# Mingqj/OcRFDet

Measured on AMD Instinct MI355X. Metric: BEV voxels/sec + rendered views/sec, 6-cam 256x704, higher is better.
Workload: dtype f32

## Files before the change

ocrfdet_amd/csrc/common.hip:

```cpp
#include <hip/hip_runtime.h>

#include <mutex>
#include <vector>

#include "launch.h"
#include "ocrf_hip.h"

namespace {

struct Timer {
  int kernel_id = 0;
  std::vector<hipEvent_t> start, stop;
  int used = 0;
};

std::mutex g_mu;
std::vector<Timer*> g_armed;
volatile int g_n_armed = 0;

}

namespace {

__global__ void zero_words_kernel(unsigned* __restrict__ dst, size_t n_words) {
  const size_t i = (size_t)blockIdx.x * blockDim.x + threadIdx.x;
  if (i < n_words) dst[i] = 0u;
}

__global__ void diag_stamp_kernel(unsigned long long* __restrict__ slot) { *slot = wall_clock64(); }

__global__ void diag_where_kernel(unsigned* __restrict__ out, int spin) {
  unsigned xcc, hw;
  asm volatile("s_getreg_b32 %0, hwreg(HW_REG_XCC_ID)" : "=s"(xcc));
  asm volatile("s_getreg_b32 %0, hwreg(HW_REG_HW_ID)" : "=s"(hw));
  const unsigned long long t0 = wall_clock64();
  while (wall_clock64() - t0 < (unsigned long long)spin) __builtin_amdgcn_s_sleep(8);
  if (threadIdx.x == 0) out[blockIdx.x] = ((xcc & 0xFu) << 16) | (hw & 0xFFFFu);
}

}

namespace ocrf {

hipError_t zero_async(void* dst, size_t bytes, hipStream_t stream) {
  const size_t n = bytes / 4;
  if (n == 0) return hipSuccess;
  hipLaunchKernelGGL(zero_words_kernel, dim3((unsigned)((n + 255) / 256)), dim3(256), 0, stream,
                     static_cast<unsigned*>(dst), n);
  return hipGetLastError();
}

bool timer_next(int kernel_id, hipEvent_t* start, hipEvent_t* stop) {
  if (!g_n_armed) return false;
  std::lock_guard<std::mutex> lk(g_mu);
  for (Timer* t : g_armed) {
    if (t->kernel_id != kernel_id || t->used >= (int)t->start.size()) continue;
    *start = t->start[t->used];
    *stop = t->stop[t->used];
    ++t->used;
    return true;
  }
  return false;
}

}

extern "C" {

const char* ocrf_version(void) { return "ocrf_hip 0.1 gfx950"; }

int ocrf_diag_stamp(unsigned long long* slot, void* stream) {
  hipLaunchKernelGGL(diag_stamp_kernel, dim3(1), dim3(1), 0, static_cast<hipStream_t>(stream), slot);
  return (int)hipGetLastError();
}

int ocrf_diag_where(int n_blocks, unsigned* out, int spin_ticks, void* stream) {
  if (n_blocks <= 0 || !out) return (int)hipErrorInvalidValue;
  hipLaunchKernelGGL(diag_where_kernel, dim3(n_blocks), dim3(64), 0, static_cast<hipStream_t>(stream), out, spin_ticks);
  return (int)hipGetLastError();
}

const char* ocrf_kernel_name(int kernel_id) {
  switch (kernel_id) {
    case OCRF_K_BEV_POOL_FWD: return "bev_pool_tile_kernel<false>";
    case OCRF_K_BEV_POOL_INTERVAL: return "bev_pool_interval_kernel";
    case OCRF_K_BEV_POOL_MFMA: return "bev_pool_mfma_kernel<*>";
    case OCRF_K_BEV_POOL_PANEL: return "bev_pool_panel_kernel<*>";
    case OCRF_K_BEV_POOL_CELL_WEIGHTS: return "bev_pool_cell_weights_kernel";
    case OCRF_K_BEV_POOL_GRAD: return "bev_pool_grad_vec_kernel";
    case OCRF_K_RASTER_PREPROCESS: return "raster_preprocess_kernel";
    case OCRF_K_RASTER_BLEND: return "raster_blend_kernel<false, false, *>";
    case OCRF_K_RASTER_BLEND_BWD: return "raster_blend_kernel<false, true, true>";
    case OCRF_K_RASTER_PRE_BWD: return "raster_preprocess_backward_kernel<false>";
    case OCRF_K_RASTER_GATHER: return "raster_scatter_kernel";
    case OCRF_K_RASTER_PLAN_UPDATE: return "raster_plan_update_kernel";
    case OCRF_K_RASTER_BLEND_SORTED: return "raster_blend_sorted_kernel<*>";
    case OCRF_K_RASTER_SCAN: return "raster_bucket_scan_kernel";
    case OCRF_K_HOA_STATS: return "hoa_channel_stats_kernel";
    case OCRF_K_HOA_MASK_GATE: return "hoa_mask_gate_kernel";
    case OCRF_K_HOA_HEIGHT_MAX: return "hoa_height_max_kernel";
    case OCRF_K_HOA_HEIGHT_GATE: return "hoa_height_gate_kernel";
    case OCRF_K_HOA_UNET_BLOCK: return "hoa_unet_block_kernel";
    case OCRF_K_HOA_OUT_CONV: return "hoa_gated_conv1x1_kernel";
    case OCRF_K_HOA1_ATTN: return "hoa1_attention_upsample_kernel";
    case OCRF_K_HOA1_UP: return "(unused)";
    case OCRF_K_HOA1_Q: return "(unused)";
    case OCRF_K_HOA1_KV: return "hoa1_kv_kernel";
    case OCRF_K_HOA_DW3X3: return "hoa_dw3x3_kernel";
    case OCRF_K_HOA_DW3X3_WGRAD: return "hoa_dw3x3_wgrad_kernel";
    case OCRF_K_LSS_KEYS: return "lss_keys_hist_kernel";
    case OCRF_K_RADIX_HIST: return "radix_hist_kernel";
    case OCRF_K_SCAN: return "scan_apply_kernel<*>";
    case OCRF_K_RADIX_SCATTER: return "radix_scatter_kernel<*>";
    case OCRF_K_LSS_BOUNDS: return "lss_intervals_kernel";
    case OCRF_K_LSS_EMIT: return "(unused)";
    case OCRF_K_HT_COUNT: return "ht_valid_kernel";
    case OCRF_K_HT_EMIT: return "ht_emit_kernel";
    case OCRF_K_HT_PROJECT: return "ht_project_kernel";
    case OCRF_K_NECK_PREFILTER: return "neck_prefilter_kernel";
    case OCRF_K_NECK_SAMPLE: return "neck_pillar_sample_mean_kernel<*>";
    case OCRF_K_NECK_RETAIN: return "neck_retain_scatter_kernel";
    case OCRF_K_NECK_HEADS: return "neck_gauss_heads_kernel";
    case OCRF_K_NECK_NERF_ALPHA: return "neck_nerf_alpha_kernel";
    case OCRF_K_NECK_NERF_RENDER: return "neck_nerf_render_kernel";
    case OCRF_K_NECK_FUSION: return "neck_dual_fusion_kernel<*>";
    case OCRF_K_NECK_PLANE_PASS: return "neck_plane_pass_kernel<*>";
    case OCRF_K_NECK_CHANNEL_MLP: return "neck_channel_mlp_kernel";
    case OCRF_K_NECK_SCALED_STATS: return "neck_scaled_channel_stats_kernel";
    case OCRF_K_NECK_CBAM_TAIL: return "neck_cbam_tail_kernel";
    case OCRF_K_LOSS_DEPTH_LABELS: return "depth_labels_kernel";
    case OCRF_K_LOSS_DS: return "ds_loss_partial_kernel";
    case OCRF_K_LOSS_FINAL: return "ds_loss_final_kernel / render_final_kernel";
    case OCRF_K_LOSS_DS_BWD: return "ds_loss_backward_kernel";
    case OCRF_K_LOSS_RENDER: return "render_tile_kernel";
    case OCRF_K_LOSS_RENDER_DEPTH: return "render_depth_kernel";
    case OCRF_K_LOSS_RENDER_BWD: return "render_backward_kernel";
    case OCRF_K_STEREO_COST_VOLUME: return "stereo_cost_volume_kernel";
    case OCRF_K_CH_ASSIGN: return "ch_assign_kernel";
    case OCRF_K_CH_HEATMAP: return "ch_heatmap_kernel";
    case OCRF_K_CH_HM_LOSS: return "ch_hm_loss_partial_kernel";
    case OCRF_K_CH_FINAL: return "ch_hm_loss_final_kernel / ch_reg_loss_final_kernel";
    case OCRF_K_CH_HM_LOSS_BWD: return "ch_hm_loss_backward_kernel";
    case OCRF_K_CH_REG_LOSS: return "ch_reg_loss_partial_kernel";
    case OCRF_K_CH_REG_LOSS_BWD: return "ch_reg_loss_backward_kernel";
    case OCRF_K_CD_SELECT: return "cd_select_kernel";
    case OCRF_K_CD_MASK: return "cd_mask_kernel";
    case OCRF_K_CD_SCAN: return "cd_scan_kernel";
    case OCRF_K_CD_WRITE: return "cd_write_kernel";
    case OCRF_K_UPSAMPLE_CAT: return "upsample_cat_kernel<float, *>";
    case OCRF_K_UPSAMPLE_CAT_BWD: return "upsample_cat_backward_kernel<float>";
    case OCRF_K_ADD_RELU: return "binary_kernel<*, AddRelu>";
    case OCRF_K_ADD_RELU_BWD: return "binary_kernel<*, Threshold>";
    case OCRF_K_UPSAMPLE_ADD: return "upsample_add_kernel<*>";
    case OCRF_K_UPSAMPLE_ADD_BWD: return "upsample_add_backward_kernel";
    case OCRF_K_BEV_ALIGN: return "bev_align_kernel<float, *>";
    case OCRF_K_BEV_ALIGN_BWD: return "bev_align_backward_kernel<float>";
    case OCRF_K_OPTIM_SQNORM: return "optim_grad_sqnorm_kernel";
    case OCRF_K_OPTIM_NORM_FINAL: return "optim_norm_final_kernel";
    case OCRF_K_OPTIM_STEP: return "optim_step_kernel";
    case OCRF_K_ADD_RELU_BF16: return "binary_bf16_kernel<*, AddRelu>";
    case OCRF_K_ADD_RELU_BWD_BF16: return "binary_bf16_kernel<*, Threshold>";
    case OCRF_K_UPSAMPLE_ADD_BF16: return "upsample_add_bf16_kernel<*>";
    case OCRF_K_UPSAMPLE_ADD_BWD_BF16: return "upsample_add_backward_bf16_kernel";
    case OCRF_K_UPSAMPLE_CAT_BF16: return "upsample_cat_kernel<unsigned short, *>";
    case OCRF_K_UPSAMPLE_CAT_BWD_BF16: return "upsample_cat_backward_kernel<unsigned short>";
    case OCRF_K_BEV_ALIGN_BF16: return "bev_align_kernel<unsigned short, *>";
    case OCRF_K_BEV_ALIGN_BWD_BF16: return "bev_align_backward_kernel<unsigned short>";
    case OCRF_K_STEREO_PACK_BF16: return "stereo_pack_bf16_kernel";
    case OCRF_K_STEREO_COST_VOLUME_BF16: return "stereo_cost_volume_bf16_kernel";
    case OCRF_K_BN_STATS: return "bn_stats_kernel<float, *>";
    case OCRF_K_BN_FINALIZE: return "bn_finalize_kernel";
    case OCRF_K_BN_ACT_FWD: return "bn_act_forward_kernel<float, *>";
    case OCRF_K_BN_ACT_BWD_REDUCE: return "bn_act_backward_reduce_kernel<float, *>";
    case OCRF_K_BN_ACT_BWD: return "bn_act_backward_kernel<float, *>";
    case OCRF_K_BN_STATS_BF16: return "bn_stats_kernel<unsigned short, *>";
    case OCRF_K_BN_ACT_FWD_BF16: return "bn_act_forward_kernel<unsigned short, *>";
    case OCRF_K_BN_ACT_BWD_REDUCE_BF16: return "bn_act_backward_reduce_kernel<unsigned short, *>";
    case OCRF_K_BN_ACT_BWD_BF16: return "bn_act_backward_kernel<unsigned short, *>";
    case OCRF_K_FRAME_POSES: return "frame_poses_kernel";
    case OCRF_K_IMAGE_PREP_HORIZONTAL: return "image_prep_horizontal_kernel";
    case OCRF_K_IMAGE_PREP_VERTICAL: return "image_prep_vertical_kernel";
    case OCRF_K_IMAGE_PREP_EPILOGUE: return "image_prep_epilogue_kernel";
    case OCRF_K_POINT_LABELS_MARK: return "point_labels_mark_kernel";
    case OCRF_K_POINT_LABELS_RESOLVE: return "point_labels_resolve_kernel";
    case OCRF_K_DEFORM_IM2COL: return "deform_im2col_kernel";
    case OCRF_K_DEFORM_COL2IM: return "deform_col2im_kernel";
    case OCRF_K_GROUP_CORR: return "group_corr_forward_kernel<*>";
    case OCRF_K_GROUP_CORR_GRAD_LEFT: return "group_corr_grad_left_kernel<*>";
    case OCRF_K_GROUP_CORR_GRAD_RIGHT: return "group_corr_grad_right_kernel<*>";
    case OCRF_K_KD_PARTIAL: return "kd_partial_kernel";
    case OCRF_K_KD_FINAL: return "kd_final_kernel";
    case OCRF_K_KD_BWD: return "kd_backward_kernel";
    case OCRF_K_RASTER_BLEND_BWD_DEPTH: return "raster_blend_kernel<false, true, true, true, true>";
    case OCRF_K_RASTER_PRE_BWD_DEPTH: return "raster_preprocess_backward_kernel<true>";
    case OCRF_K_HOA1_ATTN_TRAIN: return "hoa1_attention_train_kernel";
    case OCRF_K_HOA1_UP_GRAD: return "hoa1_up_grad_kernel";
    case OCRF_K_HOA1_ATTN_GRAD: return "hoa1_attn_grad_kernel";
    case OCRF_K_HOA1_KV_GRAD: return "hoa1_kv_grad_kernel";
    case OCRF_K_HOA1_TOKEN_GRAD: return "hoa1_token_grad_kernel";
    case OCRF_K_HOA1_PIXEL_GRAD: return "hoa1_pixel_grad_kernel";
    case OCRF_K_HOA1_WEIGHT_SUM: return "hoa1_weight_sum_kernel";
    default: return "";
  }
}

int ocrf_timer_create(int capacity, void** timer_out) {
  if (capacity <= 0 || !timer_out) return (int)hipErrorInvalidValue;
  Timer* t = new Timer();
  t->start.resize(capacity);
  t->stop.resize(capacity);
  for (int i = 0; i < capacity; ++i) {
    hipError_t e = hipEventCreate(&t->start[i]);
    if (e == hipSuccess) e = hipEventCreate(&t->stop[i]);
    if (e != hipSuccess) { delete t; return (int)e; }
  }
  *timer_out = t;
  return 0;
}

int ocrf_timer_arm(void* timer, int kernel_id) {
  std::lock_guard<std::mutex> lk(g_mu);
  Timer* t = static_cast<Timer*>(timer);
  if (!t) {
    g_armed.clear();
  } else {
    t->kernel_id = kernel_id;
    t->used = 0;
    bool present = false;
    for (Timer* q : g_armed) present = present || (q == t);
    if (!present) g_armed.push_back(t);
  }
  g_n_armed = (int)g_armed.size();
  return 0;
}

int ocrf_timer_read(void* timer, float* ms_out, int capacity, int* count_out) {
  Timer* t = static_cast<Timer*>(timer);
  if (!t || !count_out) return (int)hipErrorInvalidValue;
  int n = 0;
  {
    std::lock_guard<std::mutex> lk(g_mu);
    n = t->used;
  }
  if (n > capacity) n = capacity;
  for (int i = 0; i < n; ++i) {
    hipError_t e = hipEventSynchronize(t->stop[i]);
    if (e == hipSuccess) e = hipEventElapsedTime(&ms_out[i], t->start[i], t->stop[i]);
    if (e != hipSuccess) return (int)e;
  }
  *count_out = n;
  return 0;
}

int ocrf_stream_create(const uint32_t* cu_mask, int n_words, int priority, void** stream_out) {
  if (!stream_out || n_words < 0) return (int)hipErrorInvalidValue;
  hipStream_t s = nullptr;
  hipError_t e;
  if (cu_mask && n_words > 0) {
    e = hipExtStreamCreateWithCUMask(&s, (uint32_t)n_words, cu_mask);
  } else {
    e = hipStreamCreateWithPriority(&s, hipStreamNonBlocking, priority);
  }
  if (e != hipSuccess) return (int)e;
  *stream_out = s;
  return 0;
}

int ocrf_stream_write_value32(int* ptr, int value, ocrf_stream_t stream) {
  if (!ptr) return (int)hipErrorInvalidValue;
  return (int)hipStreamWriteValue32(static_cast<hipStream_t>(stream), ptr, (uint32_t)value, 0);
}

int ocrf_graph_node_census(void* graph, int* n_kernel, int* n_memset, int* n_memcpy, int* n_other) {
  if (!graph || !n_kernel || !n_memset || !n_memcpy || !n_other) return (int)hipErrorInvalidValue;
  size_t n = 0;
  hipError_t e = hipGraphGetNodes(static_cast<hipGraph_t>(graph), nullptr, &n);
  if (e != hipSuccess) return (int)e;
  std::vector<hipGraphNode_t> nodes(n);
  if (n) {
    e = hipGraphGetNodes(static_cast<hipGraph_t>(graph), nodes.data(), &n);
    if (e != hipSuccess) return (int)e;
  }
  *n_kernel = *n_memset = *n_memcpy = *n_other = 0;
  for (size_t i = 0; i < n; ++i) {
    hipGraphNodeType t;
    e = hipGraphNodeGetType(nodes[i], &t);
    if (e != hipSuccess) return (int)e;
    if (t == hipGraphNodeTypeKernel) ++*n_kernel;
    else if (t == hipGraphNodeTypeMemset) ++*n_memset;
    else if (t == hipGraphNodeTypeMemcpy) ++*n_memcpy;
    else ++*n_other;
  }
  return 0;
}

int ocrf_stream_destroy(void* stream) {
  return stream ? (int)hipStreamDestroy(static_cast<hipStream_t>(stream)) : 0;
}

int ocrf_timer_destroy(void* timer) {
  Timer* t = static_cast<Timer*>(timer);
  if (!t) return 0;
  {
    std::lock_guard<std::mutex> lk(g_mu);
    for (size_t i = 0; i < g_armed.size(); ++i)
      if (g_armed[i] == t) { g_armed.erase(g_armed.begin() + i); break; }
    g_n_armed = (int)g_armed.size();
  }
  for (auto e : t->start) (void)hipEventDestroy(e);
  for (auto e : t->stop) (void)hipEventDestroy(e);
  delete t;
  return 0;
}

}
```

ocrfdet_amd/csrc/hoa.hip:

```cpp
#include <hip/hip_runtime.h>

#include <algorithm>

#include "hoa1_common.h"
#include "launch.h"
#include "ocrf_hip.h"

namespace {

constexpr int kBlock = 256;
int g_mg_groups = 0, g_mg_threads = kBlock, g_stats_threads = kBlock;

__device__ __forceinline__ float sigmoidf_(float v) { return 1.0f / (1.0f + __expf(-v)); }

__global__ __launch_bounds__(kBlock) void hoa_channel_stats_kernel(const float* __restrict__ x, int C,
                                                                   long plane, float* __restrict__ stats) {
  OCRF_MAIN_CHAIN_PRIO();
  const long pix = (long)blockIdx.x * blockDim.x + threadIdx.x;
  const int b = blockIdx.y;
  if (pix >= plane) return;
  const float* p = x + (long)b * C * plane + pix;
  float sum = 0.f, mx = -INFINITY;
  int c = 0;
  for (; c + 16 <= C; c += 16) {
    float v[16];
#pragma unroll
    for (int u = 0; u < 16; ++u) v[u] = p[(long)(c + u) * plane];
#pragma unroll
    for (int u = 0; u < 16; ++u) {
      sum += v[u];
      mx = fmaxf(mx, v[u]);
    }
  }
  for (; c < C; ++c) {
    const float v = p[(long)c * plane];
    sum += v;
    mx = fmaxf(mx, v);
  }
  stats[((long)b * 2 + 0) * plane + pix] = sum / (float)C;
  stats[((long)b * 2 + 1) * plane + pix] = mx;
}

template <int VEC, int KT, bool FAST = false>
__global__ __launch_bounds__(kBlock) void hoa_mask_gate_kernel(
    const float* __restrict__ x, const float* __restrict__ stats, const float* __restrict__ opacity_bev,
    const float* __restrict__ conv_w, int k_rt, int C, int Y, int X, int groups, int n_rows,
    float* __restrict__ mask, float* __restrict__ gated) {
  OCRF_MAIN_CHAIN_PRIO();
  const int k = KT ? KT : k_rt;
  const int nt = (int)blockDim.x;
  extern __shared__ __attribute__((aligned(16))) float s_dyn[];
  const int r = k / 2, tw = FAST ? X + 8 : ((VEC == 4) ? ((X + k - 1 + 3) & ~3) : (X + k - 1));
  constexpr int PL = FAST ? 1 : 0;
  float* s_w = s_dyn;
  float* s_s = s_dyn + ((VEC == 4) ? ((2 * k * k + 3) & ~3) : 2 * k * k);
  const long plane = (long)Y * X;
  const int b = blockIdx.z / groups, g = blockIdx.z % groups;
  const long p0 = (long)blockIdx.x * nt * VEC;
  const int row0 = (int)(p0 / X) - r;
  for (int i = threadIdx.x; i < 2 * k * k; i += nt) s_w[i] = conv_w[i];
  const long pix_e = p0 + (long)threadIdx.x * VEC;
  const int cpg_e = (C + groups - 1) / groups;
  const int c0_e = g * cpg_e, c1_e = min(C, c0_e + cpg_e);
  float4 first[5];
  const bool pre = (VEC == 4) && gated && pix_e < plane && c0_e + 5 <= c1_e;
  if constexpr (VEC == 4) {
    if (pre) {
      const float* pe = x + (long)b * C * plane + pix_e;
#pragma unroll
      for (int u = 0; u < 5; ++u) first[u] = *reinterpret_cast<const float4*>(pe + (long)(c0_e + u) * plane);
    }
  }
  if constexpr (FAST) {
    const int n_items = 2 * n_rows * 64, x4 = X >> 2;
    float4* s_s4 = reinterpret_cast<float4*>(s_s);
    const int tw4 = tw >> 2;
    for (int i0 = 0; i0 < n_items; i0 += 8 * nt) {
      float4 v[8];
#pragma unroll
      for (int u = 0; u < 8; ++u) {
        const int i = min(i0 + u * nt + (int)threadIdx.x, n_items - 1);
        const int rp = i >> 6, c4 = min(i & 63, x4 - 1);
        const int ch = rp >= n_rows ? 1 : 0, y = row0 + rp - ch * n_rows;
        v[u] = *reinterpret_cast<const float4*>(stats + ((long)b * 2 + ch) * plane + (long)min(max(y, 0), Y - 1) * X + 4 * c4);
      }
#pragma unroll
      for (int u = 0; u < 8; ++u) {
        const int i = i0 + u * nt + (int)threadIdx.x;
        const int rp = i >> 6, c4 = i & 63;
        const int ch = rp >= n_rows ? 1 : 0, y = row0 + rp - ch * n_rows;
        const bool in = y >= 0 && y < Y;
        if (i < n_items && c4 < x4) s_s4[rp * tw4 + 1 + c4] = in ? v[u] : make_float4(0.f, 0.f, 0.f, 0.f);
      }
    }
    for (int i = threadIdx.x; i < 2 * n_rows * 2; i += nt)
      s_s4[(i >> 1) * tw4 + ((i & 1) ? 1 + x4 : 0)] = make_float4(0.f, 0.f, 0.f, 0.f);
  } else {
  const int n_stage = 2 * n_rows * tw;
  for (int i0 = 0; i0 < n_stage; i0 += 8 * nt) {
    float v[8];
#pragma unroll
    for (int u = 0; u < 8; ++u) {
      const int i = i0 + u * nt + threadIdx.x;
      const int ch = i / (n_rows * tw), rem = i % (n_rows * tw);
      const int y = row0 + rem / tw, xx = rem % tw - r;
      v[u] = (i < n_stage && y >= 0 && y < Y && xx >= 0 && xx < X)
                 ? stats[((long)b * 2 + ch) * plane + (long)y * X + xx] : 0.f;
    }
#pragma unroll
    for (int u = 0; u < 8; ++u) {
      const int i = i0 + u * nt + threadIdx.x;
      if (i < n_stage) s_s[i] = v[u];
    }
  }
  }
  __syncthreads();
  const long pix = p0 + (long)threadIdx.x * VEC;
  if (pix >= plane) return;
  const int yy = (int)(pix / X), xx = (int)(pix % X);
  const int ly = yy - row0 - r;
  float acc[VEC];
#pragma unroll
  for (int e = 0; e < VEC; ++e) acc[e] = 0.f;
  if constexpr (KT > 0) {
#pragma unroll
    for (int ch = 0; ch < 2; ++ch) {
#pragma unroll
      for (int i = 0; i < KT; ++i) {
        const float* row = s_s + (ch * n_rows + ly + i) * tw + xx;
        const float* wr = s_w + (ch * KT + i) * KT;
        float win[(KT + VEC - 1 + 3) & ~3];
        if constexpr (VEC == 4) {
          const float4* row4 = reinterpret_cast<const float4*>(row);
#pragma unroll
          for (int j = 0; j < (KT + VEC - 1 + 3) / 4; ++j) {
            const float4 q4 = row4[j];
            win[4 * j] = q4.x; win[4 * j + 1] = q4.y; win[4 * j + 2] = q4.z; win[4 * j + 3] = q4.w;
          }
        } else {
#pragma unroll
          for (int j = 0; j < KT + VEC - 1; ++j) win[j] = row[j];
        }
#pragma unroll
        for (int j = 0; j < KT; ++j) {
          const float w = wr[j];
#pragma unroll
          for (int e = 0; e < VEC; ++e) acc[e] = fmaf(win[j + e + PL], w, acc[e]);
        }
      }
    }
  } else {
    for (int ch = 0; ch < 2; ++ch)
      for (int i = 0; i < k; ++i) {
        const float* row = s_s + (ch * n_rows + ly + i) * tw + xx;
        const float* wr = s_w + (ch * k + i) * k;
        for (int j = 0; j < k; ++j) {
          const float w = wr[j];
#pragma unroll
          for (int e = 0; e < VEC; ++e) acc[e] = fmaf(row[j + e], w, acc[e]);
        }
      }
  }
  float m[VEC];
#pragma unroll
  for (int e = 0; e < VEC; ++e) m[e] = sigmoidf_(acc[e] + opacity_bev[(long)b * plane + pix + e]);
  if (g == 0) {
#pragma unroll
    for (int e = 0; e < VEC; ++e) mask[(long)b * plane + pix + e] = m[e];
  }
  if (gated) {
    const int cpg = (C + groups - 1) / groups;
    const int c0 = g * cpg, c1 = min(C, c0 + cpg);
    const float* p = x + (long)b * C * plane + pix;
    float* q = gated + (long)b * C * plane + pix;
    if constexpr (VEC == 4) {
      int c = c0;
      if (pre) {
#pragma unroll
        for (int u = 0; u < 5; ++u)
          *reinterpret_cast<float4*>(q + (long)(c + u) * plane) =
              make_float4(first[u].x * m[0], first[u].y * m[1], first[u].z * m[2], first[u].w * m[3]);
        c += 5;
      }
      for (; c + 5 <= c1; c += 5) {
        float4 v[5];
#pragma unroll
        for (int u = 0; u < 5; ++u) v[u] = *reinterpret_cast<const float4*>(p + (long)(c + u) * plane);
#pragma unroll
        for (int u = 0; u < 5; ++u)
          *reinterpret_cast<float4*>(q + (long)(c + u) * plane) =
              make_float4(v[u].x * m[0], v[u].y * m[1], v[u].z * m[2], v[u].w * m[3]);
      }
      for (; c < c1; ++c) {
        const float4 v = *reinterpret_cast<const float4*>(p + (long)c * plane);
        *reinterpret_cast<float4*>(q + (long)c * plane) = make_float4(v.x * m[0], v.y * m[1], v.z * m[2], v.w * m[3]);
      }
    } else {
      int c = c0;
      for (; c + 10 <= c1; c += 10) {
        float v[10];
#pragma unroll
        for (int u = 0; u < 10; ++u) v[u] = p[(long)(c + u) * plane];
#pragma unroll
        for (int u = 0; u < 10; ++u) q[(long)(c + u) * plane] = v[u] * m[0];
      }
      for (; c < c1; ++c) q[(long)c * plane] = p[(long)c * plane] * m[0];
    }
  }
}

__global__ __launch_bounds__(kBlock) void hoa_height_max_kernel(const float* __restrict__ x, long plane,
                                                                int n_split, float* __restrict__ partial) {
  __shared__ float s_m[kBlock / 64];
  const long bc = blockIdx.y;
  const float* p = x + bc * plane;
  const long chunk = (plane + n_split - 1) / n_split;
  const long lo = (long)blockIdx.x * chunk, hi = min(lo + chunk, plane);
  float m = -INFINITY;
  for (long i = lo + threadIdx.x; i < hi; i += kBlock) m = fmaxf(m, p[i]);
  for (int off = 32; off > 0; off >>= 1) m = fmaxf(m, __shfl_down(m, off));
  if ((threadIdx.x & 63) == 0) s_m[threadIdx.x >> 6] = m;
  __syncthreads();
  if (threadIdx.x == 0) {
    for (int w = 1; w < kBlock / 64; ++w) m = fmaxf(m, s_m[w]);
    partial[bc * n_split + blockIdx.x] = m;
  }
}

__global__ __launch_bounds__(kBlock) void hoa_height_gate_kernel(
    const float* __restrict__ x, int C, int hid, long plane, int n_split, const float* __restrict__ partial,
    const float* __restrict__ w1, const float* __restrict__ w2, float* __restrict__ gate,
    float* __restrict__ gated) {
  __shared__ float s_max[64];
  __shared__ float s_hid[64];
  __shared__ float s_gate[64];
  const int b = blockIdx.y, tid = threadIdx.x;
  const int q = C / 4;
  if (tid < C) {
    float m = -INFINITY;
    for (int s = 0; s < n_split; ++s) m = fmaxf(m, partial[((long)b * C + tid) * n_split + s]);
    s_max[tid] = m;
  }
  __syncthreads();
  if (tid < 4 * hid) {
    const int g = tid / hid, h = tid % hid;
    float a = 0.f;
    for (int i = 0; i < q; ++i) a = fmaf(w1[(g * hid + h) * q + i], s_max[g * q + i], a);
    s_hid[tid] = fmaxf(a, 0.f);
  }
  __syncthreads();
  if (tid < C) {
    const int g = tid / q, o = tid % q;
    float a = 0.f;
    for (int h = 0; h < hid; ++h) a = fmaf(w2[(g * q + o) * hid + h], s_hid[g * hid + h], a);
    const float gt = sigmoidf_(a);
    s_gate[tid] = gt;
    if (blockIdx.x == 0) gate[(long)b * C + tid] = gt;
  }
  __syncthreads();
  if (!gated) return;
  const long pix = (long)blockIdx.x * kBlock + tid;
  if (pix >= plane) return;
  const float* p = x + (long)b * C * plane + pix;
  float* o = gated + (long)b * C * plane + pix;
  for (int c = 0; c < C; ++c) o[(long)c * plane] = p[(long)c * plane] * s_gate[c];
}

constexpr int kDwBand = 16;
__global__ __launch_bounds__(kBlock) void hoa_dw3x3_kernel(const float* __restrict__ x, const float* __restrict__ w,
                                                           const float* __restrict__ bias, int C, int Y, int X,
                                                           float* __restrict__ y) {
  const int bc = blockIdx.z, c = bc % C;
  const int xx = blockIdx.x * 64 + (threadIdx.x & 63), yy = blockIdx.y * 4 + (threadIdx.x >> 6);
  if (xx >= X || yy >= Y) return;
  const float* p = x + (long)bc * Y * X;
  float acc = bias ? bias[c] : 0.f;
#pragma unroll
  for (int i = 0; i < 3; ++i) {
    const int sy = yy + i - 1;
    if (sy < 0 || sy >= Y) continue;
#pragma unroll
    for (int j = 0; j < 3; ++j) {
      const int sx = xx + j - 1;
      if (sx < 0 || sx >= X) continue;
      acc = fmaf(w[c * 9 + i * 3 + j], p[(long)sy * X + sx], acc);
    }
  }
  y[(long)bc * Y * X + (long)yy * X + xx] = acc;
}

__global__ __launch_bounds__(kBlock) void hoa_dw3x3_wgrad_kernel(const float* __restrict__ x,
                                                                 const float* __restrict__ dy, int Y, int X,
                                                                 float* __restrict__ partial) {
  __shared__ float s_acc[kBlock / 64][10];
  const int bc = blockIdx.y, band = blockIdx.x;
  const float* px = x + (long)bc * Y * X;
  const float* pg = dy + (long)bc * Y * X;
  const int y0 = band * kDwBand, y1 = min(y0 + kDwBand, Y);
  float acc[10];
#pragma unroll
  for (int t = 0; t < 10; ++t) acc[t] = 0.f;
  for (int idx = threadIdx.x; idx < (y1 - y0) * X; idx += kBlock) {
    const int yy = y0 + idx / X, xx = idx % X;
    const float g = pg[(long)yy * X + xx];
    acc[9] += g;
#pragma unroll
    for (int i = 0; i < 3; ++i) {
      const int sy = yy + i - 1;
      if (sy < 0 || sy >= Y) continue;
#pragma unroll
      for (int j = 0; j < 3; ++j) {
        const int sx = xx + j - 1;
        if (sx < 0 || sx >= X) continue;
        acc[i * 3 + j] = fmaf(g, px[(long)sy * X + sx], acc[i * 3 + j]);
      }
    }
  }
#pragma unroll
  for (int t = 0; t < 10; ++t) {
    float v = acc[t];
    for (int off = 32; off > 0; off >>= 1) v += __shfl_down(v, off);
    if ((threadIdx.x & 63) == 0) s_acc[threadIdx.x >> 6][t] = v;
  }
  __syncthreads();
  if (threadIdx.x < 10) {
    float v = 0.f;
    for (int wv = 0; wv < kBlock / 64; ++wv) v += s_acc[wv][threadIdx.x];
    partial[((long)bc * gridDim.x + band) * 10 + threadIdx.x] = v;
  }
}

}

namespace ocrf {
void hoa_tune(int key, int value) {
  if (key == 20 && value >= 0) g_mg_groups = value;
  if (key == 21 && (value == 64 || value == 128 || value == 256)) g_mg_threads = value;
  if (key == 22 && (value == 64 || value == 128 || value == 256)) g_stats_threads = value;
}
}

extern "C" {

int ocrf_hoa_dw3x3(const float* x, const float* w, const float* bias, int B, int C, int Y, int X, float* y,
                   ocrf_stream_t stream_) {
  if (!x || !w || !y || B <= 0 || C <= 0 || Y <= 0 || X <= 0 || (long)B * C > 65535) return (int)hipErrorInvalidValue;
  ocrf::launch(OCRF_K_HOA_DW3X3, hoa_dw3x3_kernel, dim3((X + 63) / 64, (Y + 3) / 4, B * C), dim3(kBlock), 0,
               static_cast<hipStream_t>(stream_), x, w, bias, C, Y, X, y);
  return (int)hipGetLastError();
}

int ocrf_hoa_dw3x3_wgrad_bands(int Y) { return (Y + kDwBand - 1) / kDwBand; }

int ocrf_hoa_dw3x3_wgrad(const float* x, const float* dy, int B, int C, int Y, int X, float* partial,
                         ocrf_stream_t stream_) {
  if (!x || !dy || !partial || B <= 0 || C <= 0 || Y <= 0 || X <= 0 || (long)B * C > 65535)
    return (int)hipErrorInvalidValue;
  ocrf::launch(OCRF_K_HOA_DW3X3_WGRAD, hoa_dw3x3_wgrad_kernel, dim3(ocrf_hoa_dw3x3_wgrad_bands(Y), B * C),
               dim3(kBlock), 0, static_cast<hipStream_t>(stream_), x, dy, Y, X, partial);
  return (int)hipGetLastError();
}

int ocrf_hoa_channel_stats(const float* x, int B, int C, int Y, int X, float* stats, ocrf_stream_t stream_) {
  hipStream_t stream = static_cast<hipStream_t>(stream_);
  if (!x || !stats || B <= 0 || C <= 0 || Y <= 0 || X <= 0) return (int)hipErrorInvalidValue;
  const long plane = (long)Y * X;
  const int nt = g_stats_threads;
  ocrf::launch(OCRF_K_HOA_STATS, hoa_channel_stats_kernel, dim3((unsigned)((plane + nt - 1) / nt), B), dim3(nt), 0, stream,
               x, C, plane, stats);
  return (int)hipGetLastError();
}

int ocrf_hoa_opacity_mask_gate(const float* x, const float* stats, const float* opacity_bev,
                               const float* conv_w, int k, int B, int C, int Y, int X, float* mask,
                               float* gated, ocrf_stream_t stream_) {
  hipStream_t stream = static_cast<hipStream_t>(stream_);
  if (!x || !stats || !opacity_bev || !conv_w || !mask || k <= 0 || (k & 1) == 0 || k > 15 || B <= 0 ||
      C <= 0 || Y <= 0 || X <= 0)
    return (int)hipErrorInvalidValue;
  const long plane = (long)Y * X;
  const bool vec4 = (X % 4 == 0) && ((reinterpret_cast<uintptr_t>(x) | reinterpret_cast<uintptr_t>(gated)) & 15u) == 0 &&
                    (X + 6) * 14 * 2 * 4 <= 60 * 1024;
  const int threads = g_mg_threads;
  const int per_wg = threads * (vec4 ? 4 : 1);
  const int n_rows = (per_wg + X - 2) / X + 1 + (k - 1);
  const bool fast = vec4 && k == 7 && X <= 256 && (reinterpret_cast<uintptr_t>(stats) & 15u) == 0;
  const int tw = fast ? X + 8 : (vec4 ? ((X + k - 1 + 3) & ~3) : (X + k - 1));
  const size_t lds = (size_t)((vec4 ? ((2 * k * k + 3) & ~3) : 2 * k * k) + 2 * n_rows * tw) * sizeof(float);
  if (lds > 64 * 1024) return (int)hipErrorInvalidValue;
  int groups = gated ? ((C >= 40) ? 4 : (C >= 16 ? 2 : 1)) : 1;
  if (gated && g_mg_groups > 0) groups = std::min(g_mg_groups, C);
  const dim3 grid((unsigned)((plane + per_wg - 1) / per_wg), 1, (unsigned)(B * groups));
#define OCRF_MASK_GATE(V, K, F)                                                                                       \
  ocrf::launch(OCRF_K_HOA_MASK_GATE, hoa_mask_gate_kernel<V, K, F>, grid, dim3(threads), lds, stream, x, stats, opacity_bev, \
               conv_w, k, C, Y, X, groups, n_rows, mask, gated)
  if (fast) OCRF_MASK_GATE(4, 7, true);
  else if (vec4 && k == 7) OCRF_MASK_GATE(4, 7, false);
  else if (vec4) OCRF_MASK_GATE(4, 0, false);
  else if (k == 7) OCRF_MASK_GATE(1, 7, false);
  else OCRF_MASK_GATE(1, 0, false);
#undef OCRF_MASK_GATE
  return (int)hipGetLastError();
}

size_t ocrf_hoa_height_attention_workspace_bytes(int B, int C) {
  return (size_t)B * C * 64 * sizeof(float);
}

int ocrf_hoa_height_attention(const float* x, int B, int C, int hid, int Y, int X, const float* w1,
                              const float* w2, float* gate, float* gated, void* workspace,
                              size_t workspace_bytes, ocrf_stream_t stream_) {
  hipStream_t stream = static_cast<hipStream_t>(stream_);
  if (!x || !w1 || !w2 || !gate || B <= 0 || C <= 0 || (C % 4) != 0 || C > 64 || hid <= 0 || 4 * hid > 64 ||
      Y <= 0 || X <= 0 || !workspace || workspace_bytes < ocrf_hoa_height_attention_workspace_bytes(B, C))
    return (int)hipErrorInvalidValue;
  const long plane = (long)Y * X;
  int n_split = (int)((plane + 4095) / 4096);
  if (n_split > 64) n_split = 64;
  float* partial = static_cast<float*>(workspace);
  ocrf::launch(OCRF_K_HOA_HEIGHT_MAX, hoa_height_max_kernel, dim3(n_split, B * C), dim3(kBlock), 0, stream, x,
               plane, n_split, partial);
  hipError_t e = hipGetLastError();
  if (e != hipSuccess) return (int)e;
  const unsigned gx = gated ? (unsigned)((plane + kBlock - 1) / kBlock) : 1u;
  ocrf::launch(OCRF_K_HOA_HEIGHT_GATE, hoa_height_gate_kernel, dim3(gx, B), dim3(kBlock), 0, stream, x, C, hid,
               plane, n_split, static_cast<const float*>(partial), w1, w2, gate, gated);
  return (int)hipGetLastError();
}

}

namespace {

constexpr int kUT = 16;
constexpr int kUH = kUT + 2;
constexpr int kUMaxC = 16;

struct UnetBlockArgs {
  const float* src0; const float* gate0; int C0, H0, W0; int mode;
  const float* up_w; const float* up_b; int Cup;
  const float* src1; const float* gate1; int C1;
  const float* dw_w; const float* dw_b;
  const float* pw_w; const float* pw_b; int Cout;
  const float* addend;
  float* out; float* partial_max; int H, W, tiles_x, tiles_y;
};

__device__ __forceinline__ void load_gate_dev(int b, int C, const float* gate_vec, float* s_gate) {
  if ((int)threadIdx.x < C) s_gate[threadIdx.x] = gate_vec ? gate_vec[b * C + threadIdx.x] : 1.f;
  __syncthreads();
}

__global__ __launch_bounds__(kBlock) void hoa_unet_block_kernel(UnetBlockArgs a) {
  __shared__ float s_v[kUMaxC][kUH][kUH + 1];
  __shared__ float s_red[kBlock / 64][kUMaxC];
  __shared__ float s_upw[kUMaxC * kUMaxC * 4], s_upb[kUMaxC], s_dww[kUMaxC * 9], s_dwb[kUMaxC],
      s_pww[kUMaxC * kUMaxC], s_pwb[kUMaxC], s_g0[kUMaxC], s_g1[kUMaxC];
  const int tid = threadIdx.x;
  {
    const int Cf = (a.mode == 2) ? a.Cup : a.C0, Ci = Cf + a.C1;
    if (a.mode == 2) {
      for (int i = tid; i < a.C0 * a.Cup * 4; i += kBlock) s_upw[i] = a.up_w[i];
      if (tid < a.Cup) s_upb[tid] = a.up_b[tid];
    }
    for (int i = tid; i < Ci * 9; i += kBlock) s_dww[i] = a.dw_w[i];
    for (int i = tid; i < a.Cout * Ci; i += kBlock) s_pww[i] = a.pw_w[i];
    if (tid < Ci) s_dwb[tid] = a.dw_b[tid];
    if (tid < a.Cout) s_pwb[tid] = a.pw_b[tid];
  }
  __syncthreads();
  load_gate_dev(blockIdx.z, a.C0, a.gate0, s_g0);
  if (a.C1 > 0) load_gate_dev(blockIdx.z, a.C1, a.gate1, s_g1);
  const int b = blockIdx.z;
  const int ty0 = blockIdx.y * kUT, tx0 = blockIdx.x * kUT;
  const int Cfirst = (a.mode == 2) ? a.Cup : a.C0;
  const int Cin = Cfirst + a.C1;
  const int H = a.H, W = a.W;

  for (int i = tid; i < kUH * kUH; i += kBlock) {
    const int hy = i / kUH, hx = i % kUH;
    const int y = ty0 + hy - 1, x = tx0 + hx - 1;
    const bool in = (y >= 0) && (y < H) && (x >= 0) && (x < W);
    float sv[kUMaxC];
    if (a.mode == 2) {
      const int sy = in ? (y >> 1) : 0, sx = in ? (x >> 1) : 0, ki = (y & 1) * 2 + (x & 1);
#pragma unroll
      for (int ci = 0; ci < kUMaxC; ++ci)
        sv[ci] = (in && ci < a.C0) ? a.src0[(((long)b * a.C0 + ci) * a.H0 + sy) * a.W0 + sx] * s_g0[ci] : 0.f;
      float acc[kUMaxC];
#pragma unroll
      for (int co = 0; co < kUMaxC; ++co) acc[co] = (co < a.Cup) ? s_upb[co] : 0.f;
#pragma unroll
      for (int ci = 0; ci < kUMaxC; ++ci) {
        if (ci < a.C0) {
#pragma unroll
          for (int co = 0; co < kUMaxC; ++co)
            if (co < a.Cup) acc[co] = fmaf(sv[ci], s_upw[(ci * a.Cup + co) * 4 + ki], acc[co]);
        }
      }
#pragma unroll
      for (int co = 0; co < kUMaxC; ++co)
        if (co < a.Cup) s_v[co][hy][hx] = in ? acc[co] : 0.f;
    } else if (a.mode == 1) {
#pragma unroll
      for (int c = 0; c < kUMaxC; ++c) {
        float v = 0.f;
        if (in && c < a.C0) {
          const float* q = a.src0 + ((long)b * a.C0 + c) * a.H0 * a.W0 + (long)(2 * y) * a.W0 + 2 * x;
          v = fmaxf(fmaxf(q[0], q[1]), fmaxf(q[a.W0], q[a.W0 + 1])) * s_g0[c];
        }
        sv[c] = v;
      }
#pragma unroll
      for (int c = 0; c < kUMaxC; ++c)
        if (c < a.C0) s_v[c][hy][hx] = sv[c];
    } else {
#pragma unroll
      for (int c = 0; c < kUMaxC; ++c)
        sv[c] = (in && c < a.C0) ? a.src0[((long)b * a.C0 + c) * a.H0 * a.W0 + (long)y * a.W0 + x] * s_g0[c] : 0.f;
#pragma unroll
      for (int c = 0; c < kUMaxC; ++c)
        if (c < a.C0) s_v[c][hy][hx] = sv[c];
    }
    for (int c = 0; c < a.C1; ++c) {
      float v = 0.f;
      if (in) {
        v = a.src1[(((long)b * a.C1 + c) * H + y) * W + x] * s_g1[c];
      }
      s_v[Cfirst + c][hy][hx] = v;
    }
  }
  __syncthreads();

  const int ly = tid / kUT, lx = tid % kUT;
  const int y = ty0 + ly, x = tx0 + lx;
  const bool valid = (y < H) && (x < W);
  float outv[kUMaxC];
#pragma unroll
  for (int co = 0; co < kUMaxC; ++co) outv[co] = (co < a.Cout) ? s_pwb[co] : 0.f;
  for (int c = 0; c < Cin; ++c) {
    float d = s_dwb[c];
#pragma unroll
    for (int i = 0; i < 3; ++i)
#pragma unroll
      for (int j = 0; j < 3; ++j) d = fmaf(s_v[c][ly + i][lx + j], s_dww[c * 9 + i * 3 + j], d);
#pragma unroll
    for (int co = 0; co < kUMaxC; ++co)
      if (co < a.Cout) outv[co] = fmaf(d, s_pww[co * Cin + c], outv[co]);
  }
  const long plane = (long)H * W;
  const long pix = (long)y * W + x;
#pragma unroll
  for (int co = 0; co < kUMaxC; ++co) {
    if (co < a.Cout) {
      float v = fmaxf(outv[co], 0.f);
      if (valid) {
        if (a.addend) v += a.addend[((long)b * a.Cout + co) * plane + pix];
        a.out[((long)b * a.Cout + co) * plane + pix] = v;
      } else {
        v = -INFINITY;
      }
      outv[co] = v;
    }
  }
  if (a.partial_max) {
#pragma unroll
    for (int co = 0; co < kUMaxC; ++co) {
      if (co < a.Cout) {
        float m = outv[co];
        for (int off = 32; off > 0; off >>= 1) m = fmaxf(m, __shfl_down(m, off));
        if ((tid & 63) == 0) s_red[tid >> 6][co] = m;
      }
    }
    __syncthreads();
    if (tid < a.Cout) {
      float m = s_red[0][tid];
      for (int w = 1; w < kBlock / 64; ++w) m = fmaxf(m, s_red[w][tid]);
      const int n_tiles = a.tiles_x * a.tiles_y;
      a.partial_max[((long)b * a.Cout + tid) * n_tiles + blockIdx.y * a.tiles_x + blockIdx.x] = m;
    }
  }
}

__global__ __launch_bounds__(kBlock) void hoa_height_gate_from_tiles_kernel(
    int C, int hid, int n_tiles, const float* __restrict__ partial, const float* __restrict__ w1,
    const float* __restrict__ w2, float* __restrict__ gate) {
  __shared__ float s_max[64];
  __shared__ float s_hid[64];
  const int b = blockIdx.x, tid = threadIdx.x;
  const int wave = tid >> 6, lane = tid & 63;
  const int q = C / 4;
  for (int c = wave; c < C; c += kBlock / 64) {
    float m = -INFINITY;
    for (int t = lane; t < n_tiles; t += 64) m = fmaxf(m, partial[((long)b * C + c) * n_tiles + t]);
    for (int off = 32; off > 0; off >>= 1) m = fmaxf(m, __shfl_down(m, off));
    if (lane == 0) s_max[c] = m;
  }
  __syncthreads();
  if (tid < 4 * hid) {
    const int g = tid / hid, h = tid % hid;
    float acc = 0.f;
    for (int i = 0; i < q; ++i) acc = fmaf(w1[(g * hid + h) * q + i], s_max[g * q + i], acc);
    s_hid[tid] = fmaxf(acc, 0.f);
  }
  __syncthreads();
  if (tid < C) {
    const int g = tid / q, o = tid % q;
    float acc = 0.f;
    for (int h = 0; h < hid; ++h) acc = fmaf(w2[(g * q + o) * hid + h], s_hid[g * hid + h], acc);
    gate[(long)b * C + tid] = sigmoidf_(acc);
  }
}

__global__ __launch_bounds__(kBlock) void hoa_gated_conv1x1_kernel(const float* __restrict__ x,
                                                                   const float* __restrict__ gate, int C,
                                                                   long plane, const float* __restrict__ w,
                                                                   const float* __restrict__ bias,
                                                                   float* __restrict__ out) {
  __shared__ float s_g[64];
  const int b = blockIdx.y;
  load_gate_dev(b, C, gate, s_g);
  const long pix = (long)blockIdx.x * kBlock + threadIdx.x;
  if (pix >= plane) return;
  float acc = bias[0];
  for (int c = 0; c < C; ++c) acc = fmaf(x[((long)b * C + c) * plane + pix] * s_g[c], w[c], acc);
  out[(long)b * plane + pix] = acc;
}

}

extern "C" {

int ocrf_hoa_unet_block(const float* src0, const float* gate0, int C0, int H0, int W0, int mode,
                        const float* up_w, const float* up_b, int Cup, const float* src1,
                        const float* gate1, int C1, const float* dw_w, const float* dw_b,
                        const float* pw_w, const float* pw_b, int Cout, const float* addend, float* out,
                        float* partial_max, int B, int H, int W, ocrf_stream_t stream_) {
  hipStream_t stream = static_cast<hipStream_t>(stream_);
  const int Cfirst = (mode == 2) ? Cup : C0;
  if (!src0 || !dw_w || !dw_b || !pw_w || !pw_b || !out || B <= 0 || H <= 0 || W <= 0 || mode < 0 || mode > 2 ||
      C0 <= 0 || C0 > kUMaxC || C1 < 0 || Cfirst + C1 > kUMaxC || Cout <= 0 || Cout > kUMaxC ||
      (mode == 2 && (!up_w || !up_b || Cup <= 0)) || (C1 > 0 && !src1))
    return (int)hipErrorInvalidValue;
  if ((mode == 0 && (H0 != H || W0 != W)) || (mode == 1 && (H0 / 2 != H || W0 / 2 != W)) ||
      (mode == 2 && (H0 * 2 != H || W0 * 2 != W)))
    return (int)hipErrorInvalidValue;
  UnetBlockArgs a;
  a.src0 = src0; a.gate0 = gate0; a.C0 = C0; a.H0 = H0; a.W0 = W0; a.mode = mode;
  a.up_w = up_w; a.up_b = up_b; a.Cup = Cup; a.src1 = src1; a.gate1 = gate1; a.C1 = C1;
  a.dw_w = dw_w; a.dw_b = dw_b; a.pw_w = pw_w; a.pw_b = pw_b; a.Cout = Cout; a.addend = addend;
  a.out = out; a.partial_max = partial_max; a.H = H; a.W = W;
  a.tiles_x = (W + kUT - 1) / kUT; a.tiles_y = (H + kUT - 1) / kUT;
  ocrf::launch(OCRF_K_HOA_UNET_BLOCK, hoa_unet_block_kernel, dim3(a.tiles_x, a.tiles_y, B), dim3(kBlock), 0, stream, a);
  return (int)hipGetLastError();
}


int ocrf_hoa_unet_tiles(int H, int W) { return ((W + kUT - 1) / kUT) * ((H + kUT - 1) / kUT); }

int ocrf_hoa_height_gate_from_tiles(int B, int C, int hid, int n_tiles, const float* partial_max,
                                    const float* w1, const float* w2, float* gate, ocrf_stream_t stream_) {
  hipStream_t stream = static_cast<hipStream_t>(stream_);
  if (!partial_max || !w1 || !w2 || !gate || B <= 0 || C <= 0 || (C % 4) || C > 64 || hid <= 0 || 4 * hid > 64 ||
      n_tiles <= 0)
    return (int)hipErrorInvalidValue;
  ocrf::launch(OCRF_K_HOA_HEIGHT_GATE, hoa_height_gate_from_tiles_kernel, dim3(B), dim3(kBlock), 0, stream, C, hid,
               n_tiles, partial_max, w1, w2, gate);
  return (int)hipGetLastError();
}

int ocrf_hoa_gated_conv1x1(const float* x, const float* gate, int B, int C, int H, int W, const float* w,
                           const float* bias, float* out, ocrf_stream_t stream_) {
  hipStream_t stream = static_cast<hipStream_t>(stream_);
  if (!x || !gate || !w || !bias || !out || B <= 0 || C <= 0 || H <= 0 || W <= 0) return (int)hipErrorInvalidValue;
  const long plane = (long)H * W;
  ocrf::launch(OCRF_K_HOA_OUT_CONV, hoa_gated_conv1x1_kernel, dim3((unsigned)((plane + kBlock - 1) / kBlock), B),
               dim3(kBlock), 0, stream, x, gate, C, plane, w, bias, out);
  return (int)hipGetLastError();
}

}

namespace {

using namespace ocrf::hoa1;
static_assert(kHoaBlock == kBlock, "the HOA-1 kernels are written for 256 threads");

__global__ __launch_bounds__(kBlock) void hoa1_kv_kernel(const float* __restrict__ opacity,
                                                         const float* __restrict__ alpha,
// ... 297 lines not shown
```

Before: 388.9 million.

## Add single-pass mask-gate kernel computing each pixel's conv once per block

Adds a new mask-gate kernel, on by default for the vec4 path. Each block owns a run of pixels and computes the 7x7 (or k×k) opacity conv once per pixel, storing the mask in LDS. All 256 threads then stream the channels as float4 and multiply by the shared mask, instead of splitting channels into groups that each redo the conv and stat staging. The channel loads for the first batch are issued before the stat staging to hide latency. The LDS staging code moves into a shared helper. This removes the repeated conv and stats staging per channel group, at the cost of more registers for the prefetch (10 float4 per thread) and fewer blocks.

Result: no change. 393.4 million (median of 4 runs) (+1.2%).

```diff
diff --git a/ocrfdet_amd/csrc/common.hip b/ocrfdet_amd/csrc/common.hip
--- a/ocrfdet_amd/csrc/common.hip
+++ b/ocrfdet_amd/csrc/common.hip
@@ -97,7 +97,7 @@
     case OCRF_K_RASTER_BLEND_SORTED: return "raster_blend_sorted_kernel<*>";
     case OCRF_K_RASTER_SCAN: return "raster_bucket_scan_kernel";
     case OCRF_K_HOA_STATS: return "hoa_channel_stats_kernel";
-    case OCRF_K_HOA_MASK_GATE: return "hoa_mask_gate_kernel";
+    case OCRF_K_HOA_MASK_GATE: return "hoa_mask_gate*_kernel";
     case OCRF_K_HOA_HEIGHT_MAX: return "hoa_height_max_kernel";
     case OCRF_K_HOA_HEIGHT_GATE: return "hoa_height_gate_kernel";
     case OCRF_K_HOA_UNET_BLOCK: return "hoa_unet_block_kernel";
diff --git a/ocrfdet_amd/csrc/hoa.hip b/ocrfdet_amd/csrc/hoa.hip
--- a/ocrfdet_amd/csrc/hoa.hip
+++ b/ocrfdet_amd/csrc/hoa.hip
@@ -10,6 +10,7 @@
 
 constexpr int kBlock = 256;
 int g_mg_groups = 0, g_mg_threads = kBlock, g_stats_threads = kBlock;
+int g_mg_once = 1, g_mg_run = 256;
 
 __device__ __forceinline__ float sigmoidf_(float v) { return 1.0f / (1.0f + __expf(-v)); }
 
@@ -39,6 +40,56 @@
   }
   stats[((long)b * 2 + 0) * plane + pix] = sum / (float)C;
   stats[((long)b * 2 + 1) * plane + pix] = mx;
+}
+
+template <bool FAST, int U>
+__device__ __forceinline__ void hoa_stage_stat_rows(const float* __restrict__ stats, int b, int Y, int X, int r, int tw,
+                                                    int row0, int n_rows, float* __restrict__ s_s) {
+  const int nt = (int)blockDim.x;
+  const long plane = (long)Y * X;
+  if constexpr (FAST) {
+    const int n_items = 2 * n_rows * 64, x4 = X >> 2;
+    float4* s_s4 = reinterpret_cast<float4*>(s_s);
+    const int tw4 = tw >> 2;
+    for (int i0 = 0; i0 < n_items; i0 += U * nt) {
+      float4 v[U];
+#pragma unroll
+      for (int u = 0; u < U; ++u) {
+        const int i = min(i0 + u * nt + (int)threadIdx.x, n_items - 1);
+        const int rp = i >> 6, c4 = min(i & 63, x4 - 1);
+        const int ch = rp >= n_rows ? 1 : 0, y = row0 + rp - ch * n_rows;
+        v[u] = *reinterpret_cast<const float4*>(stats + ((long)b * 2 + ch) * plane + (long)min(max(y, 0), Y - 1) * X + 4 * c4);
+      }
+#pragma unroll
+      for (int u = 0; u < U; ++u) {
+        const int i = i0 + u * nt + (int)threadIdx.x;
+        const int rp = i >> 6, c4 = i & 63;
+        const int ch = rp >= n_rows ? 1 : 0, y = row0 + rp - ch * n_rows;
+        const bool in = y >= 0 && y < Y;
+        if (i < n_items && c4 < x4) s_s4[rp * tw4 + 1 + c4] = in ? v[u] : make_float4(0.f, 0.f, 0.f, 0.f);
+      }
+    }
+    for (int i = threadIdx.x; i < 2 * n_rows * 2; i += nt)
+      s_s4[(i >> 1) * tw4 + ((i & 1) ? 1 + x4 : 0)] = make_float4(0.f, 0.f, 0.f, 0.f);
+  } else {
+    const int n_stage = 2 * n_rows * tw;
+    for (int i0 = 0; i0 < n_stage; i0 += U * nt) {
+      float v[U];
+#pragma unroll
+      for (int u = 0; u < U; ++u) {
+        const int i = i0 + u * nt + threadIdx.x;
+        const int ch = i / (n_rows * tw), rem = i % (n_rows * tw);
+        const int y = row0 + rem / tw, xx = rem % tw - r;
+        v[u] = (i < n_stage && y >= 0 && y < Y && xx >= 0 && xx < X)
+                   ? stats[((long)b * 2 + ch) * plane + (long)y * X + xx] : 0.f;
+      }
+#pragma unroll
+      for (int u = 0; u < U; ++u) {
+        const int i = i0 + u * nt + threadIdx.x;
+        if (i < n_stage) s_s[i] = v[u];
+      }
+    }
+  }
 }
 
 template <int VEC, int KT, bool FAST = false>
@@ -71,49 +122,7 @@
       for (int u = 0; u < 5; ++u) first[u] = *reinterpret_cast<const float4*>(pe + (long)(c0_e + u) * plane);
     }
   }
-  if constexpr (FAST) {
-    const int n_items = 2 * n_rows * 64, x4 = X >> 2;
-    float4* s_s4 = reinterpret_cast<float4*>(s_s);
-    const int tw4 = tw >> 2;
-    for (int i0 = 0; i0 < n_items; i0 += 8 * nt) {
-      float4 v[8];
-#pragma unroll
-      for (int u = 0; u < 8; ++u) {
-        const int i = min(i0 + u * nt + (int)threadIdx.x, n_items - 1);
-        const int rp = i >> 6, c4 = min(i & 63, x4 - 1);
-        const int ch = rp >= n_rows ? 1 : 0, y = row0 + rp - ch * n_rows;
-        v[u] = *reinterpret_cast<const float4*>(stats + ((long)b * 2 + ch) * plane + (long)min(max(y, 0), Y - 1) * X + 4 * c4);
-      }
-#pragma unroll
-      for (int u = 0; u < 8; ++u) {
-        const int i = i0 + u * nt + (int)threadIdx.x;
-        const int rp = i >> 6, c4 = i & 63;
-        const int ch = rp >= n_rows ? 1 : 0, y = row0 + rp - ch * n_rows;
-        const bool in = y >= 0 && y < Y;
-        if (i < n_items && c4 < x4) s_s4[rp * tw4 + 1 + c4] = in ? v[u] : make_float4(0.f, 0.f, 0.f, 0.f);
-      }
-    }
-    for (int i = threadIdx.x; i < 2 * n_rows * 2; i += nt)
-      s_s4[(i >> 1) * tw4 + ((i & 1) ? 1 + x4 : 0)] = make_float4(0.f, 0.f, 0.f, 0.f);
-  } else {
-  const int n_stage = 2 * n_rows * tw;
-  for (int i0 = 0; i0 < n_stage; i0 += 8 * nt) {
-    float v[8];
-#pragma unroll
-    for (int u = 0; u < 8; ++u) {
-      const int i = i0 + u * nt + threadIdx.x;
-      const int ch = i / (n_rows * tw), rem = i % (n_rows * tw);
-      const int y = row0 + rem / tw, xx = rem % tw - r;
-      v[u] = (i < n_stage && y >= 0 && y < Y && xx >= 0 && xx < X)
-                 ? stats[((long)b * 2 + ch) * plane + (long)y * X + xx] : 0.f;
-    }
-#pragma unroll
-    for (int u = 0; u < 8; ++u) {
-      const int i = i0 + u * nt + threadIdx.x;
-      if (i < n_stage) s_s[i] = v[u];
-    }
-  }
-  }
+  hoa_stage_stat_rows<FAST, 8>(stats, b, Y, X, r, tw, row0, n_rows, s_s);
   __syncthreads();
   const long pix = p0 + (long)threadIdx.x * VEC;
   if (pix >= plane) return;
@@ -206,6 +215,81 @@
       }
       for (; c < c1; ++c) q[(long)c * plane] = p[(long)c * plane] * m[0];
     }
+  }
+}
+
+template <int KT, bool FAST>
+__global__ __launch_bounds__(kBlock) void hoa_mask_gate_once_kernel(
+    const float* __restrict__ x, const float* __restrict__ stats, const float* __restrict__ opacity_bev,
+    const float* __restrict__ conv_w, int k_rt, int C, int Y, int X, int run, int n_rows,
+    float* __restrict__ mask, float* __restrict__ gated) {
+  OCRF_MAIN_CHAIN_PRIO();
+  constexpr int NP = 10;
+  constexpr int PL = FAST ? 1 : 0;
+  const int k = KT ? KT : k_rt;
+  extern __shared__ __attribute__((aligned(16))) float s_dyn[];
+  const int r = k / 2, tw = FAST ? X + 8 : ((X + k - 1 + 3) & ~3);
+  float* s_m = s_dyn;
+  float* s_w = s_dyn + run;
+  float* s_s = s_w + (KT ? 0 : ((2 * k * k + 3) & ~3));
+  const long plane = (long)Y * X;
+  const int b = blockIdx.z, tid = threadIdx.x;
+  const long p0 = (long)blockIdx.x * run;
+  const int row0 = (int)(p0 / X) - r;
+  const int sh = __ffs(run) - 3;
+  const int q = tid & ((run >> 2) - 1), cl = tid >> sh, ncl = kBlock >> sh;
+  const long pix_q = p0 + 4 * q;
+  const bool live = gated && pix_q < plane;
+  const float* px = x + (long)b * C * plane + pix_q;
+  float4 v[NP];
+  if (live) {
+#pragma unroll
+    for (int u = 0; u < NP; ++u)
+      if (cl + u * ncl < C) v[u] = *reinterpret_cast<const float4*>(px + (long)(cl + u * ncl) * plane);
+  }
+  const long pix_m = p0 + tid;
+  const bool conv = tid < run && pix_m < plane;
+  const float ob = conv ? opacity_bev[(long)b * plane + pix_m] : 0.f;
+  if constexpr (KT == 0)
+    for (int i = tid; i < 2 * k * k; i += kBlock) s_w[i] = conv_w[i];
+  hoa_stage_stat_rows<FAST, 4>(stats, b, Y, X, r, tw, row0, n_rows, s_s);
+  __syncthreads();
+  if (conv) {
+    const int yy = (int)(pix_m / X), xx = (int)(pix_m % X);
+    const float* win = s_s + (yy - row0 - r) * tw + xx + PL;
+    float acc = 0.f;
+    if constexpr (KT > 0) {
+#pragma unroll
+      for (int ch = 0; ch < 2; ++ch)
+#pragma unroll
+        for (int i = 0; i < KT; ++i)
+#pragma unroll
+          for (int j = 0; j < KT; ++j) acc = fmaf(win[(ch * n_rows + i) * tw + j], conv_w[(ch * KT + i) * KT + j], acc);
+    } else {
+      for (int ch = 0; ch < 2; ++ch)
+        for (int i = 0; i < k; ++i)
+          for (int j = 0; j < k; ++j) acc = fmaf(win[(ch * n_rows + i) * tw + j], s_w[(ch * k + i) * k + j], acc);
+    }
+    const float m = sigmoidf_(acc + ob);
+    s_m[tid] = m;
+    mask[(long)b * plane + pix_m] = m;
+  }
+  if (!gated) return;
+  __syncthreads();
+  if (!live) return;
+  const float4 m = *reinterpret_cast<const float4*>(s_m + 4 * q);
+  float* pq = gated + (long)b * C * plane + pix_q;
+  for (int c0 = cl;;) {
+#pragma unroll
+    for (int u = 0; u < NP; ++u)
+      if (c0 + u * ncl < C)
+        *reinterpret_cast<float4*>(pq + (long)(c0 + u * ncl) * plane) =
+            make_float4(v[u].x * m.x, v[u].y * m.y, v[u].z * m.z, v[u].w * m.w);
+    c0 += NP * ncl;
+    if (c0 >= C) break;
+#pragma unroll
+    for (int u = 0; u < NP; ++u)
+      if (c0 + u * ncl < C) v[u] = *reinterpret_cast<const float4*>(px + (long)(c0 + u * ncl) * plane);
   }
 }
 
@@ -337,6 +421,8 @@
   if (key == 20 && value >= 0) g_mg_groups = value;
   if (key == 21 && (value == 64 || value == 128 || value == 256)) g_mg_threads = value;
   if (key == 22 && (value == 64 || value == 128 || value == 256)) g_stats_threads = value;
+  if (key == 23 && (value == 64 || value == 128 || value == 256)) g_mg_run = value;
+  if (key == 24 && (value == 0 || value == 1)) g_mg_once = value;
 }
 }
 
@@ -381,10 +467,25 @@
   const long plane = (long)Y * X;
   const bool vec4 = (X % 4 == 0) && ((reinterpret_cast<uintptr_t>(x) | reinterpret_cast<uintptr_t>(gated)) & 15u) == 0 &&
                     (X + 6) * 14 * 2 * 4 <= 60 * 1024;
+  const bool fast = vec4 && k == 7 && X <= 256 && (reinterpret_cast<uintptr_t>(stats) & 15u) == 0;
+  if (vec4 && g_mg_once) {
+    const int run = g_mg_run, n_rows = (run + X - 2) / X + 1 + (k - 1);
+    const int tw = fast ? X + 8 : ((X + k - 1 + 3) & ~3);
+    const size_t lds = (size_t)(run + (k == 7 ? 0 : ((2 * k * k + 3) & ~3)) + 2 * n_rows * tw) * sizeof(float);
+    if (lds > 64 * 1024) return (int)hipErrorInvalidValue;
+    const dim3 grid((unsigned)((plane + run - 1) / run), 1, (unsigned)B);
+#define OCRF_MASK_GATE_ONCE(K, F)                                                                                     \
+  ocrf::launch(OCRF_K_HOA_MASK_GATE, hoa_mask_gate_once_kernel<K, F>, grid, dim3(kBlock), lds, stream, x, stats,      \
+               opacity_bev, conv_w, k, C, Y, X, run, n_rows, mask, gated)
+    if (fast) OCRF_MASK_GATE_ONCE(7, true);
+    else if (k == 7) OCRF_MASK_GATE_ONCE(7, false);
+    else OCRF_MASK_GATE_ONCE(0, false);
+#undef OCRF_MASK_GATE_ONCE
+    return (int)hipGetLastError();
+  }
   const int threads = g_mg_threads;
   const int per_wg = threads * (vec4 ? 4 : 1);
   const int n_rows = (per_wg + X - 2) / X + 1 + (k - 1);
-  const bool fast = vec4 && k == 7 && X <= 256 && (reinterpret_cast<uintptr_t>(stats) & 15u) == 0;
   const int tw = fast ? X + 8 : (vec4 ? ((X + k - 1 + 3) & ~3) : (X + k - 1));
   const size_t lds = (size_t)((vec4 ? ((2 * k * k + 3) & ~3) : 2 * k * k) + 2 * n_rows * tw) * sizeof(float);
   if (lds > 64 * 1024) return (int)hipErrorInvalidValue;
```
